# LeoIV/polyaxon

Hardware: AMD Instinct MI355X
Metric: HPO trials/hour (whole node) + wall-clock-to-target, ResNet-50 Hyperband sweep (higher is better)
Workload: dtype bf16

## Files before the change

polyaxon_amd/csrc/conv_gemm.hip:

```cpp
#include <hip/hip_runtime.h>

#include <stdint.h>

namespace {

typedef __bf16 bf16x8 __attribute__((ext_vector_type(8)));
typedef short s16x4 __attribute__((ext_vector_type(4)));
typedef float f32x4 __attribute__((ext_vector_type(4)));
typedef uint32_t u32x4 __attribute__((ext_vector_type(4)));
typedef __attribute__((address_space(3))) void lds_void;
typedef __attribute__((address_space(1))) const void gbl_void;

constexpr int BK = 64;

struct ConvGeom {
    int H, W;
    int Hr, Wr;
    int C, S, ntaps;
    int Hc, Wc, OS, oph, opw;
    signed char offh[9], offw[9], btap[9];
    int tap_a[9], tap_b[9];
    uint32_t mWr, mHr;
    int nh, nw, hv[3], wv[3];
    uint32_t pat[9];
    int tap_inner;
};

__device__ __forceinline__ int pick9(const int (&v)[9], int t) {
    int r = v[0];
#pragma unroll
    for (int i = 1; i < 9; ++i) r = t == i ? v[i] : r;
    return r;
}

inline uint32_t div_magic(int d) { return d <= 1 ? 0u : (uint32_t)((1ull << 32) / (unsigned)d + 1); }
// ... 606 lines not shown
    }
    if (stats_on) {
        float* pa = stats + (size_t)srow * N + n0;
        float* pb = stats + (size_t)(nsr + srow) * N + n0;
        reduce_store(s1, s2, pa, pb);
        zero_rows(pa, pb, N);
    }
}

template <int ROWB>
__device__ __forceinline__ int tr_swz(int row) {
    if constexpr (ROWB >= 256) return 2 * ((row & 3) | (((row >> 3) & 1) << 2));
    else return 2 * (((row >> 1) & 1) | (((row >> 3) & 1) << 1));
}

template <int ROWB>
__device__ __forceinline__ s16x4 tr_read(const char* img, int row, int col ) {
    const int lc = col >> 3, half = (col >> 2) & 1;
    const int pc = lc ^ tr_swz<ROWB>(row);
    return __builtin_amdgcn_ds_read_tr16_b64_v4i16(
        (__attribute__((address_space(3))) s16x4*)(img + row * ROWB + pc * 16 + half * 8));
}

__device__ __forceinline__ uint32_t lds_addr(const void* p) {
    return (uint32_t)(uintptr_t)(const __attribute__((address_space(3))) char*)p;
}

__device__ __forceinline__ s16x4 ds_tr(uint32_t addr) {
    s16x4 r;
    asm volatile("ds_read_b64_tr_b16 %0, %1" : "=v"(r) : "v"(addr) : "memory");
    return r;
}

template <int ROWB, int GATHER = 0, int BKR = BK>
__device__ __forceinline__ void stage_rows(char* img, __amdgpu_buffer_rsrc_t rsrc, int ld, int r0, int rend, int c0,
                                           int wave, int lane, const ConvGeom* geo = nullptr, int dh = 0, int dw = 0) {
    constexpr int INSTR = BKR * ROWB / 1024;
    static_assert(INSTR % 4 == 0, "a stage splits evenly over the 4 waves");
#pragma unroll
    for (int i = 0; i < INSTR / 4; ++i) {
        const int off = (i * 4 + wave) * 1024 + lane * 16;
        const int row = off / ROWB, pc = (off % ROWB) >> 4;
        const int lc = pc ^ tr_swz<ROWB>(row);
        const int gr = r0 + row;
        uint32_t boff;
        if constexpr (GATHER == 2) {
            int n, r, c;
            row_coords(gr, *geo, n, r, c);
            const int t = (c0 >> 3) + lc, ih = 2 * r - 3 + (t >> 2), sc = c - 2 + (t & 3);
            const bool ok = gr < rend && t < 28 && (unsigned)ih < (unsigned)geo->H && (unsigned)sc < (unsigned)geo->W;
            boff = ok ? (uint32_t)(((n * geo->H + ih) * geo->W + sc) * 16) : OOB;
        } else if constexpr (GATHER == 1) {
            int n, r, c;
            row_coords(gr, *geo, n, r, c);
            const int ih = r * geo->S + dh, iw = c * geo->S + dw;
            const bool ok = gr < rend && (unsigned)ih < (unsigned)geo->H && (unsigned)iw < (unsigned)geo->W;
            boff = ok ? (uint32_t)(((((n * geo->H + ih) * geo->W + iw) * ld) + c0 + lc * 8) * 2) : OOB;
        } else {
            boff = gr < rend ? (uint32_t)((gr * ld + c0 + lc * 8) * 2) : OOB;
        }
        blds16(rsrc, boff, img + (i * 4 + wave) * 1024);
    }
}


template <int BN1, int BN2, int WG1, int WG2, int CONV, int NST = 2, int BKT = BK>
// ... 357 lines not shown
            const float v = red[tw * 4096 + row * 64 + (lane ^ (((row >> 2) & 3) << 4))];
            float* dst = W + (size_t)(n10 + (tw / NB) * 64 + row) * ldc + n20 + (tw % NB) * 64 + lane;
            __hip_atomic_fetch_add(dst, v, __ATOMIC_RELAXED, __HIP_MEMORY_SCOPE_AGENT);
        }
        return;
    }
    float* slab = W + (size_t)slice * N1 * N2;
#pragma unroll
    for (int a = 0; a < 4; ++a)
#pragma unroll
        for (int b = 0; b < 4; ++b) {
            const int c2 = n20 + w2 * 64 + b * 16 + gi;
            const int r1 = n10 + w1 * 64 + a * 16 + 4 * g4;
#pragma unroll
            for (int r = 0; r < 4; ++r) slab[(size_t)(r1 + r) * N2 + c2] = acc[a][b][r];
        }
}

__global__ void weight_prep_kernel(const float* __restrict__ w, __bf16* __restrict__ wb, __bf16* __restrict__ wt,
                                   int cout, int cin) {
    __shared__ float tile[32][33];
    const int c0 = blockIdx.x * 32, o0 = blockIdx.y * 32;
    const int tx = threadIdx.x & 31, ty = threadIdx.x >> 5;
    for (int j = ty; j < 32; j += 8) {
        const int o = o0 + j, c = c0 + tx;
        float v = (o < cout && c < cin) ? w[(size_t)o * cin + c] : 0.f;
        tile[j][tx] = v;
        if (o < cout && c < cin) wb[(size_t)o * cin + c] = (__bf16)v;
    }
    __syncthreads();
    for (int j = ty; j < 32; j += 8) {
        const int c = c0 + j, o = o0 + tx;
        if (o < cout && c < cin) wt[(size_t)c * cout + o] = (__bf16)tile[tx][j];
    }
}

template <typename KernelT>
int set_lds(KernelT k, int bytes) {
    return hipFuncSetAttribute((const void*)k, hipFuncAttributeMaxDynamicSharedMemorySize, bytes) == hipSuccess ? 0
                                                                                                                 : -2;
}

template <int BM, int BN, int WGM, int WGN, int CONV = 0, int NBUF = 2>
int launch_nt(const void* A, const void* B, void* C, int M, int N, int K, int lda, int ldb, int ldc, float* stats,
              hipStream_t s, ConvGeom geo = {}, const void* D = nullptr, int ldd = 0, BnBwd bnr = {},
              const uint8_t* dmask = nullptr) {
    constexpr int NTH = NTHREADS;
    constexpr int TILE = BM * (BN * 2 + 16), RED = NTH * 17 * 4;
    constexpr int EPI = TILE > RED ? TILE : RED;
    constexpr int KLOOP = NBUF * (BM + BN) * BK * 2;
    constexpr int LDS = KLOOP > EPI ? KLOOP : EPI;
    static_assert(NBUF >= 1 && NBUF <= 2, "one or two K stages");
    static_assert(NBUF == 1 || EPI <= KLOOP, "epilogue staging must fit the k-loop LDS");
    static_assert(LDS <= 160 * 1024, "LDS");
    constexpr int PER_CU = (160 * 1024) / LDS;
    constexpr int CAP = CONV != 0 && BN == 64 ? 3 : 4;
    constexpr int MIN_F = NBUF == 1 ? (PER_CU < CAP ? PER_CU : CAP) : 2, MIN_B = MIN_F;
    auto kf = gemm_nt_kernel<BM, BN, WGM, WGN, CONV, MIN_F, NBUF, false, NTH>;
    auto kb = gemm_nt_kernel<BM, BN, WGM, WGN, CONV, MIN_B, NBUF, true, NTH>;
    static int attr = set_lds(kf, LDS) | set_lds(kb, LDS);
    if (attr) return attr;
    const bool bwd = D != nullptr || bnr.part != nullptr;
    if (bwd && stats != nullptr) return -1;
    auto k = bwd ? kb : kf;
    const int nwg = ((M + BM - 1) / BM) * (N / BN);
    hipLaunchKernelGGL(k, dim3(nwg), dim3(NTH), LDS, s, (const __bf16*)A, (const __bf16*)B, (__bf16*)C, M, N,
                       K, lda, ldb, ldc, stats, geo, (const __bf16*)D, ldd, bnr, dmask, BnDx{}, BnApply{});
    return hipGetLastError() == hipSuccess ? 0 : -3;
}

template <int BM, int BN, int WGM, int WGN, bool BNDX, int BNAP>
int launch_nt_prod(const void* A, const BnDx& bd, const BnApply& ba, const void* B, void* C, int M, int N, int K,
                   int ldb, int ldc, float* stats, hipStream_t s, const void* D = nullptr, int ldd = 0, BnBwd bnr = {},
                   const uint8_t* dmask = nullptr) {
    constexpr int TILE = BM * (BN * 2 + 16), RED = NTHREADS * 17 * 4;
    constexpr int LDS = 2 * (BM + BN) * BK * 2;
    static_assert(TILE <= LDS && RED <= LDS && LDS <= 80 * 1024, "epilogue staging fits; 2 blocks per CU");
    static_assert(BNDX != (BNAP != 0), "exactly one producer mode");
    auto k = gemm_nt_kernel<BM, BN, WGM, WGN, 0, 2, 2, BNDX, NTHREADS, BNDX, BNAP>;
    static int attr = set_lds(k, LDS);
    if (attr) return attr;
    const int nwg = ((M + BM - 1) / BM) * (N / BN);
    hipLaunchKernelGGL(k, dim3(nwg), dim3(NTHREADS), LDS, s, (const __bf16*)A, (const __bf16*)B, (__bf16*)C, M, N, K, K,
                       ldb, ldc, stats, ConvGeom{}, (const __bf16*)D, ldd, bnr, dmask, bd, ba);
    return hipGetLastError() == hipSuccess ? 0 : -3;
}


inline bool nt_single(bool conv, int K, int nwg) { return nwg >= 768 || (!conv && K == BK); }

inline int nt_plan(bool conv, int M, int N, int K) {
    const int bm = N % 128 == 0 ? 128 : 256, bn = N % 128 == 0 ? 128 : 64;
    return bm + 1000 * (nt_single(conv, K, ((M + bm - 1) / bm) * (N / bn)) ? 1 : 2);
}

struct TnPlan { int kchunk, slices, groups, per_group, blocks, bn1, bn2; };

inline void tn_tile(int N1, int N2, int& bn1, int& bn2) {
    bn1 = N1 % 128 == 0 ? 128 : 64;
    bn2 = N2 % 128 == 0 ? 128 : 64;
}

inline void plan_reducer(TnPlan& p, long plane) {
    const long total4 = plane / 4;
    int blocks = (int)((total4 + 255) / 256);
    if (blocks > 2048) blocks = 2048;
    int groups = 1024 / blocks;
    if (groups > p.slices / 8) groups = p.slices / 8;
    if (groups < 1) groups = 1;
    const int per_group = (p.slices + groups - 1) / groups;
    p.groups = (p.slices + per_group - 1) / per_group;
    p.per_group = per_group;
    p.blocks = blocks;
}

inline long plan_slabs(const TnPlan& p) { return p.slices + (p.groups > 1 ? p.groups : 0); }

constexpr int g_tn_bpc_big = 3, g_tn_bpc_mid = 1;
constexpr long g_tn_slab_bytes = 16l << 20;

// ... 161 lines not shown
    switch (nt_plan(false, M, N, K)) {
        case 1128:
            return launch_nt<128, 128, 2, 2, false, 1>(A, B, C, M, N, K, lda, ldb, ldc, stats, s, {}, D, ldd, b, dmask);
        case 2128:
            return launch_nt<128, 128, 2, 2>(A, B, C, M, N, K, lda, ldb, ldc, stats, s, {}, D, ldd, b, dmask);
        case 1256:
            return launch_nt<256, 64, 4, 1, false, 1>(A, B, C, M, N, K, lda, ldb, ldc, stats, s, {}, D, ldd, b, dmask);
        default:
            return launch_nt<256, 64, 4, 1>(A, B, C, M, N, K, lda, ldb, ldc, stats, s, {}, D, ldd, b, dmask);
    }
}

int plx_gemm_nt_plan(int M, int N, int K, int conv) {
    if (M <= 0 || N <= 0 || N % 64 || K <= 0 || K % BK) return -1;
    return nt_plan(conv != 0, M, N, K);
}

int plx_gemm_nt_bndx(const void* g, const void* x, const uint8_t* mask, const float* coef, void* dy, const void* Wt,
                     void* C, int M, int N, int K, int ldb, int ldc, const void* D, int ldd, const uint8_t* dmask,
                     const BnBwd* bnr, void* stream) {
    if (M <= 0 || N % 64 || K % BK || ldb % 8 || ldc % 8 || (D != nullptr && ldd % 8)) return -1;
    if (g == nullptr || x == nullptr || coef == nullptr || dy == nullptr || dy == g || dy == x) return -1;
    if ((long)M * K >= (1l << 30)) return -1;
    if (dmask != nullptr && (D == nullptr || ldd != N)) return -1;
    if (bnr != nullptr && (ldc != N || bnr->part == nullptr)) return -1;
    const BnBwd b = bnr != nullptr ? *bnr : BnBwd{};
    const BnDx bd{(const __bf16*)x, mask, coef, (__bf16*)dy};
    hipStream_t s = (hipStream_t)stream;
    if (N % 128 == 0)
        return launch_nt_prod<128, 128, 2, 2, true, 0>(g, bd, {}, Wt, C, M, N, K, ldb, ldc, nullptr, s, D, ldd, b, dmask);
    return launch_nt_prod<256, 64, 4, 1, true, 0>(g, bd, {}, Wt, C, M, N, K, ldb, ldc, nullptr, s, D, ldd, b, dmask);
}

int plx_gemm_nt_bnapply(const void* x, const void* res, const float* sb, const float* rsb, void* out, uint8_t* mask,
                        const void* W, void* C, int M, int N, int K, int ldb, int ldc, float* stats, void* stream) {
    if (M <= 0 || N % 64 || K % BK || ldb % 8 || ldc % 8) return -1;
    if (x == nullptr || res == nullptr || sb == nullptr || out == nullptr || mask == nullptr || out == x || out == res)
        return -1;
    if ((long)M * K >= (1l << 30)) return -1;
    const BnApply ba{(const __bf16*)res, sb, rsb, (__bf16*)out, mask};
    hipStream_t s = (hipStream_t)stream;
    if (N % 128 == 0)
        return rsb != nullptr ? launch_nt_prod<128, 128, 2, 2, false, 2>(x, {}, ba, W, C, M, N, K, ldb, ldc, stats, s)
                              : launch_nt_prod<128, 128, 2, 2, false, 1>(x, {}, ba, W, C, M, N, K, ldb, ldc, stats, s);
    return rsb != nullptr ? launch_nt_prod<256, 64, 4, 1, false, 2>(x, {}, ba, W, C, M, N, K, ldb, ldc, stats, s)
                          : launch_nt_prod<256, 64, 4, 1, false, 1>(x, {}, ba, W, C, M, N, K, ldb, ldc, stats, s);
}

int plx_tn_plan_slices(int M, int N1, int N2, int num_cus, int v2) {
    if (M <= 0 || N1 % 64 || N2 % 64) return -1;
    return v2 ? tn2_plan(M, N1, N2, num_cus, v2_cfg(N1, N2)).slices : tn_plan(M, N1, N2, num_cus).slices;
}

void plx_set_tn2_c64(int on) { g_tn2_c64 = on ? 1 : 0; }

void plx_set_tn_atomic(int on) { g_tn_atomic = on ? 1 : 0; }

void plx_set_tn2_stem(int mode) { g_tn2_stem = mode < 0 ? 0 : (mode > 2 ? 2 : mode); }

void plx_set_tn_v2(int on, int lds_kb) {
    g_tn_v2 = on < 0 ? 0 : (on > 2 ? 2 : on);
    if (lds_kb > 0) g_tn2_lds_kb = lds_kb <= 64 ? 64 : 128;
}

long plx_gemm_tn_workspace(int M, int N1, int N2, int num_cus) {
    if (M <= 0 || N1 % 64 || N2 % 64) return -1;
    const long a = plan_slabs(tn_plan(M, N1, N2, num_cus));
    const long b = plan_slabs(tn2_plan(M, N1, N2, num_cus, v2_cfg(N1, N2)));
    return (a > b ? a : b) * N1 * N2;
}

}

namespace {
template <int CONV>
int run_tn(const void* A, const void* B, float* C, float* ws, int M, int N1, int N2, int lda, int ldb, int ldc,
           int num_cus, int accumulate, hipStream_t s, ConvGeom geo, int bpc = 0) {
    const V2Cfg cfg = v2_cfg(N1, N2);
    const bool six = cfg.na == 1 && cfg.nb == 3;
    const bool v2 = CONV == 2 ? g_tn2_stem > 0
                              : (g_tn_v2 == 1 || (g_tn_v2 == 2 && CONV != 0)) && (!six || g_tn2_c64);
    const TnPlan plan = v2 ? tn2_plan(M, N1, N2, num_cus, cfg, CONV == 2 && g_tn2_stem == 1 ? kStemV2Bpc : 0)
                           : tn_plan(M, N1, N2, num_cus, bpc);
    int rc;
    if (v2 && g_tn_atomic) {
        if (!accumulate && hipMemset2DAsync(C, (size_t)ldc * 4, 0, (size_t)N2 * 4, N1, s) != hipSuccess) return -3;
        return dispatch_tn2<CONV>(cfg, A, B, C, M, N1, N2, lda, ldb, plan, s, geo, true, ldc);
    }
    if (v2)
// ... 330 lines not shown
```

polyaxon_amd/ops/_native.py:

```python
from __future__ import annotations

import ctypes
import hashlib
import os
import shutil
import subprocess
import threading
from pathlib import Path
from typing import Dict, Iterable, List, Optional

PKG_DIR = Path(__file__).resolve().parent.parent
CSRC = PKG_DIR / "csrc"
OUT = PKG_DIR / "_native"
ARCH = os.environ.get("PLX_OFFLOAD_ARCH", "gfx950")
ROCM = Path(os.environ.get("ROCM_PATH", "/opt/rocm"))

LIBRARIES: Dict[str, dict] = {
    "plx_train": {"sources": ["train_kernels.hip"], "kind": "hip", "link": []},
    "plx_polytune": {"sources": ["polytune_kernels.hip"], "kind": "hip", "link": []},
    "plx_bn": {"sources": ["bn_kernels.hip"], "kind": "hip", "link": []},
    "plx_procmon": {"sources": ["procmon.cpp"], "kind": "cpp", "link": ["-lpthread"]},
    "plx_gp": {"sources": ["gp_kernels.hip", "gp_chol.hip"], "kind": "hip", "link": []},
    "plx_rms": {"sources": ["rmsnorm.hip"], "kind": "hip", "link": []},
    "plx_conv": {"sources": ["conv_gemm.hip"], "kind": "hip", "link": []},
# ... 190 lines not shown
        "plx_bn_backward": [_P, _P],
        "plx_bn_dx_blocks": [_L, _I],
        "plx_stem_bn_pool_forward": [_P, _P, _P, _I, _I, _I, _I, _P, _P, _F, _F, _P, _P, _P, _P, _P, _P, _P, _I, _P,
                                     _P],
        "plx_stem_bn_pool_bwd_workspace": [_I, _I, _I, _I],
        "plx_stem_bn_pool_backward": [_P, _P, _P, _P, _I, _I, _I, _I, _P, _P, _P, _P, _P, _P, _P, _P, _I, _P, _P],
    },
    "plx_procmon": {
        "plx_pm_create": [],
        "plx_pm_destroy": [_P],
        "plx_pm_spawn": [_P, _P, _P, ctypes.c_char_p, ctypes.c_char_p, ctypes.POINTER(_I)],
        "plx_pm_wait": [_P, _I, ctypes.POINTER(_I), ctypes.POINTER(_I)],
        "plx_pm_wake": [_P],
        "plx_pm_signal": [_P, _I, _I, _I],
        "plx_pm_count": [_P],
    },
    "plx_gp": {
        "plx_gp_kmat": [_P, _P, _I, _I, _I, _P, _I, _I, _F, _F, _F, _I, _F, _P, _P, _D, _I, _P],
        "plx_gp_chol": [_P, _I, _I, _P, _P],
        "plx_gp_kmat_batch_f64": [_P, _I, _I, _P, _I, _P, _I, _L, _I, _D, _D, _D, _P, _P, _D, _I, _P],
        "plx_gp_matern_table": [_D, _D, _D, _I, _P, _P, _P],
        "plx_gp_chol_aug_f64": [_P, _I, _I, _I, _L, _I, _P, _P, _P],
        "plx_gp_chol_scratch_doubles": [],
        "plx_gp_lml_f64": [_P, _I, _I, _L, _I, _P, _P, _P],
        "plx_gp_acq_rows": [_P, _I, _I, _P, _F, _I, _F, _F, _F, _P, _P, _P, _P],
        "plx_gp_predict_acq": [_P, _I, _P, _I, _I, _P, _I, _P, _I, _F, _F, _F, _F, _I, _F, _F, _F, _P, _P, _P, _P,
                               _P, _P, _P, _D, _I, _P],
        "plx_gp_ascent": [_P, _P, _I, _P, _P, _P, _I, _I, _P, _P, _I, _F, _F, _F, _F, _I, _F, _F, _F, _I, _P, _P, _D, _I,
                          _P],
    },
    "plx_conv": {
        "plx_gemm_nt": [_P, _P, _P, _I, _I, _I, _I, _I, _I, _P, _P, _I, _P, _P, _P],
        "plx_gemm_nt_bndx": [_P, _P, _P, _P, _P, _P, _P, _I, _I, _I, _I, _I, _P, _I, _P, _P, _P],
        "plx_gemm_nt_bnapply": [_P, _P, _P, _P, _P, _P, _P, _P, _I, _I, _I, _I, _I, _P, _P],
        "plx_gemm_nt_rows_per_block": [_I],
        "plx_gemm_nt_plan": [_I, _I, _I, _I],
        "plx_gemm_tn_workspace": [_I, _I, _I, _I],
        "plx_set_tn_v2": [_I, _I],
        "plx_set_tn2_stem": [_I],
        "plx_set_tn2_c64": [_I],
        "plx_set_tn_atomic": [_I],
        "plx_tn_plan_slices": [_I, _I, _I, _I, _I],
        "plx_gemm_tn": [_P, _P, _P, _P, _I, _I, _I, _I, _I, _I, _I, _I, _P],
        "plx_weight_prep": [_P, _P, _P, _I, _I, _P],
        "plx_weight_prepk": [_P, _L, _L, _L, _L, _P, _P, _I, _I, _I, _P],
        "plx_weight_prep_all": [_P, _P, _P, _P, _I, _I, _P],
        "plx_stem_pack_input": [_P, _P, _I, _I, _I, _P],
        "plx_stem_pack_weight": [_P, _L, _L, _L, _L, _P, _I, _P],
        "plx_stem_conv_fwd": [_P, _P, _P, _I, _I, _I, _P, _P],
        "plx_stem_conv_wgrad_workspace": [_I, _I, _I, _I],
        "plx_stem_conv_wgrad": [_P, _P, _P, _L, _L, _L, _L, _P, _I, _I, _I, _I, _I, _P],
        "plx_conv_fwd": [_P, _P, _P, _I, _I, _I, _I, _I, _I, _I, _P, _P],
        "plx_conv_dgrad": [_P, _P, _P, _I, _I, _I, _I, _I, _I, _I, _P, _P, _P],
        "plx_conv_dgrad_blocks": [_I, _I, _I, _I, _I, _I, _I],
        "plx_conv_wgrad_workspace": [_I, _I, _I, _I, _I, _I, _I, _I],
        "plx_conv_wgrad": [_P, _P, _P, _P, _I, _I, _I, _I, _I, _I, _I, _I, _I, _P],
    },
    "plx_lm": {
        "plx_qkv_rope_fwd": [_P, _P, _P, _P, _P, _P, _L, _I, _I, _I, _I, _I, _P],
        "plx_qkv_rope_bwd": [_P, _P, _P, _P, _P, _P, _L, _I, _I, _I, _I, _I, _P],
        "plx_swiglu_fwd": [_P, _P, _L, _I, _P],
        "plx_swiglu_bwd": [_P, _P, _P, _L, _I, _P],
        "plx_xent_fwd": [_P, _P, _P, _P, _I, _I, _I, _P],
        "plx_xent_bwd": [_P, _P, _P, _P, _P, _I, _I, _I, _P],
        "plx_xent_cls_fwd": [_P, _P, _P, _P, _I, _I, _P],
        "plx_xent_cls_bwd": [_P, _P, _P, _P, _P, _I, _I, _F, _P],
        "plx_xent_hp_fwd": [_P, _P, _P, _P, _P, _P, _I, _I, _I, _I, _P],
        "plx_xent_hp_bwd": [_P, _P, _P, _P, _P, _P, _I, _I, _I, _I, _P],
        "plx_xent_cls_hp_fwd": [_P, _P, _P, _P, _P, _P, _I, _I, _I, _P],
        "plx_xent_cls_hp_bwd": [_P, _P, _P, _P, _P, _P, _I, _I, _I, _F, _P],
        "plx_colsum_splits": [_L, _I],
        "plx_colsum": [_P, _L, _I, _P, _P, _P, _I, _P],
        "plx_gelu_bwd_colsum": [_P, _P, _P, _L, _I, _P, _P, _P, _I, _P],
    },
# ... 107 lines not shown
```

polyaxon_amd/ops/conv1x1.py:

```python
from __future__ import annotations

import ctypes
import os
from typing import Dict

import torch
import torch.nn as nn
import torch.nn.functional as F

from polyaxon_amd.ops import _native, side_stream, wcache
from polyaxon_amd.ops.flat import direct_grad

_CUS: Dict[int, int] = {}

_BN_DX_FUSED = os.environ.get("PLX_BN_DX_FUSED", "1") != "0"


def set_bn_dx_fused(on: bool) -> bool:
    global _BN_DX_FUSED
    prev, _BN_DX_FUSED = _BN_DX_FUSED, bool(on)
    return prev


_BN_APPLY_FUSED = os.environ.get("PLX_BN_APPLY_FUSED", "1") != "0"


def set_bn_apply_fused(on: bool) -> bool:
    global _BN_APPLY_FUSED
    prev, _BN_APPLY_FUSED = _BN_APPLY_FUSED, bool(on)
    return prev


def bn_apply_fused() -> bool:
    return _BN_APPLY_FUSED


def _num_cus(dev: torch.device) -> int:
    idx = dev.index if dev.index is not None else torch.cuda.current_device()
    if idx not in _CUS:
        _CUS[idx] = torch.cuda.get_device_properties(idx).multi_processor_count
    return _CUS[idx]


def _stream() -> int:
    return _native.current_stream()


def nt_stats_rows(n: int) -> int:
    return _native.size("plx_conv", "plx_gemm_nt_rows_per_block", n)


def _check_stats(stats, m: int, n: int) -> None:
    if stats is not None:
        nblk = -(-m // nt_stats_rows(n))
        assert stats.dtype == torch.float32 and stats.is_contiguous() and stats.numel() >= 2 * nblk * n


def _check_add(add, add_mask, m: int, n: int) -> None:
    if add is not None:
        assert add.shape == (m, n) and add.stride(1) == 1 and add.dtype == torch.bfloat16 and add.data_ptr() % 16 == 0
    if add_mask is not None:
        assert add is not None and add.stride(0) == n and add_mask.dtype == torch.uint8 and add_mask.numel() == m * n // 8


def gemm_nt(a: torch.Tensor, b: torch.Tensor, out: torch.Tensor = None, stats: torch.Tensor = None,
            add: torch.Tensor = None, bnr: "_native.GemmBnBwdArgs" = None,
            add_mask: torch.Tensor = None) -> torch.Tensor:
# ... 9 lines not shown
                                             b.stride(0), out.stride(0),
                                             stats.data_ptr() if stats is not None else None,
                                             add.data_ptr() if add is not None else None,
                                             add.stride(0) if add is not None else 0,
                                             add_mask.data_ptr() if add_mask is not None else None,
                                             ctypes.addressof(bnr) if bnr is not None else None, _stream())
    _native.check(rc, "plx_gemm_nt")
    return out


def gemm_nt_bndx(g: torch.Tensor, x: torch.Tensor, mask: torch.Tensor, coef: torch.Tensor, dy: torch.Tensor,
                 b: torch.Tensor, out: torch.Tensor = None, add: torch.Tensor = None,
                 bnr: "_native.GemmBnBwdArgs" = None, add_mask: torch.Tensor = None) -> torch.Tensor:
    m, k = g.shape
    n = b.shape[0]
    if out is None:
        out = torch.empty(m, n, dtype=torch.bfloat16, device=g.device)
    for t in (g, x, dy):
        assert t.shape == (m, k) and t.dtype == torch.bfloat16 and t.stride() == (k, 1) and t.data_ptr() % 16 == 0
    assert b.stride(1) == 1 and out.stride(1) == 1 and b.shape[1] == k and b.dtype == torch.bfloat16
    assert b.data_ptr() % 16 == 0 and out.data_ptr() % 16 == 0
    assert coef.dtype == torch.float32 and coef.is_contiguous() and coef.numel() == 3 * k
    if mask is not None:
        assert mask.dtype == torch.uint8 and mask.numel() == m * k // 8
    _check_add(add, add_mask, m, n)
    rc = _native.lib("plx_conv").plx_gemm_nt_bndx(g.data_ptr(), x.data_ptr(),
                                                  mask.data_ptr() if mask is not None else None, coef.data_ptr(),
                                                  dy.data_ptr(), b.data_ptr(), out.data_ptr(), m, n, k, b.stride(0),
                                                  out.stride(0), add.data_ptr() if add is not None else None,
                                                  add.stride(0) if add is not None else 0,
                                                  add_mask.data_ptr() if add_mask is not None else None,
                                                  ctypes.addressof(bnr) if bnr is not None else None, _stream())
    _native.check(rc, "plx_gemm_nt_bndx")
    return out


def gemm_nt_bnapply(x: torch.Tensor, res: torch.Tensor, sb: torch.Tensor, rsb, out_a: torch.Tensor, mask: torch.Tensor,
                    b: torch.Tensor, out: torch.Tensor = None, stats: torch.Tensor = None) -> torch.Tensor:
    m, k = x.shape
    n = b.shape[0]
    if out is None:
        out = torch.empty(m, n, dtype=torch.bfloat16, device=x.device)
    for t in (x, res, out_a):
        assert t.shape == (m, k) and t.dtype == torch.bfloat16 and t.stride() == (k, 1) and t.data_ptr() % 16 == 0
    assert b.stride(1) == 1 and out.stride(1) == 1 and b.shape[1] == k and b.dtype == torch.bfloat16
    assert b.data_ptr() % 16 == 0 and out.data_ptr() % 16 == 0
    assert mask.dtype == torch.uint8 and mask.is_contiguous() and mask.numel() >= m * k // 8
    for c in (sb, rsb):
        assert c is None or (c.dtype == torch.float32 and c.is_contiguous() and c.numel() == 2 * k
                             and c.data_ptr() % 16 == 0)
    assert sb is not None
    _check_stats(stats, m, n)
    rc = _native.lib("plx_conv").plx_gemm_nt_bnapply(x.data_ptr(), res.data_ptr(), sb.data_ptr(),
                                                     rsb.data_ptr() if rsb is not None else None, out_a.data_ptr(),
                                                     mask.data_ptr(), b.data_ptr(), out.data_ptr(), m, n, k,
                                                     b.stride(0), out.stride(0),
                                                     stats.data_ptr() if stats is not None else None, _stream())
    _native.check(rc, "plx_gemm_nt_bnapply")
    return out


def gemm_tn(a: torch.Tensor, b: torch.Tensor, out: torch.Tensor = None, accumulate: bool = False) -> torch.Tensor:
    m, n1 = a.shape
    n2 = b.shape[1]
    if out is None:
        out = torch.empty(n1, n2, dtype=torch.float32, device=a.device)
# ... 201 lines not shown
        x = x.to(torch.bfloat16).contiguous(memory_format=torch.channels_last)
        ctx.box = box
        ctx.dxsink = dxsink
        ctx.sink = sink if (sink is not None and sink.armed) else None
        if ctx.sink is not None:
            ctx.sink.expect = True
        ctx.link = link if (sink is None or sink.armed) else None
        ctx.wgrad = direct_grad(weight)
        n, cin, h, w = x.shape
        cout = weight.shape[0]
        wb, wt = wcache.lookup(weight) or weight_prep(weight)
        y = torch.empty((n, cout, h, w), dtype=torch.bfloat16, device=x.device, memory_format=torch.channels_last)
        if pend is not None:
            gemm_nt_bnapply(_rows(pend.x), _rows(pend.res), pend.sb, pend.rsb, _rows(x), pend.mask, wb, _rows(y), stats)
            pend.release()
        else:
            gemm_nt(_rows(x), wb, _rows(y), stats)
        ctx.save_for_backward(x, wt)
        ctx.wshape = weight.shape
        ctx.wdtype = weight.dtype
        return y

    @staticmethod
    def backward(ctx, dy):
        x, wt = ctx.saved_tensors
        n, cin, h, w = x.shape
        fused = ctx.dxsink.take() if ctx.dxsink is not None else None
        if fused is not None and (dy.data_ptr() != fused[4].data_ptr() or dy.shape != fused[4].shape
                                  or dy.dtype != torch.bfloat16 or not ctx.needs_input_grad[0]):
            raise RuntimeError("DxSink: the BatchNorm's deferred input gradient was replaced before the convolution's "
                               "backward could fill it")
        dy = dy.to(torch.bfloat16).contiguous(memory_format=torch.channels_last)
        dx = dw = None
        extra, extra_mask = ctx.box.take() if ctx.box is not None else (None, None)
        if ctx.needs_input_grad[0]:
            dx = torch.empty_like(x, memory_format=torch.channels_last)
            if extra is not None and (extra.dtype != torch.bfloat16
                                      or not extra.is_contiguous(memory_format=torch.channels_last)):
                if extra_mask is not None:
                    extra, extra_mask = unpack_relu_mask(extra, extra_mask), None
                extra = extra.to(torch.bfloat16).contiguous(memory_format=torch.channels_last)
            bnr = None
            rows = nt_stats_rows(cin)
            if ctx.link is not None and ctx.sink is None and (ctx.box is None or extra is not None):
                bnr = ctx.link.request(-(-(n * h * w) // rows))
            elif ctx.link is not None and ctx.sink is not None and ctx.sink.s2k1 and extra is None:
                bnr = ctx.link.request_split(-(-(n * h * w) // rows), -(-(n * ((h + 1) // 2) * ((w + 1) // 2)) // rows))
            if fused is not None:
                g, bx, bmask, coef, _ = fused
                gemm_nt_bndx(_rows(g), _rows(bx), bmask, coef, _rows(dy), wt, _rows(dx),
                             add=_rows(extra) if extra is not None else None, bnr=bnr, add_mask=extra_mask)
            else:
                gemm_nt(_rows(dy), wt, _rows(dx), add=_rows(extra) if extra is not None else None, bnr=bnr,
                        add_mask=extra_mask)
            if ctx.sink is not None:
                ctx.sink.put(dx)
                dx = None
        if ctx.needs_input_grad[1]:
            cout = ctx.wshape[0]
            if ctx.wgrad is not None:
                slot = ctx.wgrad.as_strided((cout, cin), (cin, 1))
                side_stream.run(lambda: gemm_tn(_rows(dy), _rows(x), out=slot, accumulate=True), (dy, x), x.device)
            else:
                dw = gemm_tn(_rows(dy), _rows(x)).view(ctx.wshape).to(ctx.wdtype)
        return dx, dw, None, None, None, None, None, None


def _bf16_context(x: torch.Tensor) -> bool:
    if x.dtype == torch.bfloat16:
        return True
    return torch.is_autocast_enabled("cuda") and torch.get_autocast_dtype("cuda") == torch.bfloat16


def supported(x: torch.Tensor, conv: nn.Conv2d) -> bool:
    return (x.is_cuda and x.dim() == 4 and _bf16_context(x) and conv.kernel_size == (1, 1) and conv.stride == (1, 1)
            and conv.padding == (0, 0) and conv.groups == 1 and conv.bias is None
            and conv.in_channels % 64 == 0 and conv.out_channels % 64 == 0 and x.numel() > 0)


def conv1x1(x: torch.Tensor, weight: torch.Tensor, with_stats: bool = False,
            grad_box: "GradMailbox" = None, grad_sink: "GradMailbox" = None, bn_link: bool = False) -> torch.Tensor:
    stats = None
    if with_stats:
        n, _, h, w = x.shape
        m, cout = n * h * w, weight.shape[0]
        nblk = -(-m // nt_stats_rows(cout))
        stats = torch.empty(2 * nblk * cout, dtype=torch.float32, device=x.device)
    if grad_box is not None:
        grad_box.armed = True
    dxsink = dx_sink_for(x, weight)
    pend = getattr(x, "_plx_pending", None)
# ... 31 lines not shown
```

Before: 13000.

## Fuse weight-gradient accumulation into BN-dx producer dgrad kernel for 64-channel 1x1 convs

Adds a persistent kernel for 1x1 convs with 64 input channels. It rebuilds the BatchNorm input gradient tile once in LDS and uses it for both the data-gradient GEMM and the weight-gradient product against the saved input. The weight gradient is reduced in registers across row tiles and flushed with atomic adds into the fp32 weight-grad buffer. This removes the separate gemm_tn pass that re-read dy and x, but that pass used to run on a side stream and now runs serially inside the dgrad kernel, so the overlap is lost and the dgrad kernel does more work. It is on by default through an environment flag, but only when the atomic weight-gradient mode is enabled.

```diff
diff --git a/polyaxon_amd/csrc/conv_gemm.hip b/polyaxon_amd/csrc/conv_gemm.hip
--- a/polyaxon_amd/csrc/conv_gemm.hip
+++ b/polyaxon_amd/csrc/conv_gemm.hip
@@ -1,6 +1,8 @@
 #include <hip/hip_runtime.h>
 
 #include <stdint.h>
+
+#include <type_traits>
 
 namespace {
 
@@ -673,6 +675,14 @@
     return r;
 }
 
+template <int OFF>
+__device__ __forceinline__ s16x4 ds_tr_o(uint32_t addr) {
+    static_assert(OFF >= 0 && OFF < 65536, "16-bit offset field");
+    s16x4 r;
+    asm volatile("ds_read_b64_tr_b16 %0, %1 offset:%2" : "=v"(r) : "v"(addr), "n"(OFF) : "memory");
+    return r;
+}
+
 template <int ROWB, int GATHER = 0, int BKR = BK>
 __device__ __forceinline__ void stage_rows(char* img, __amdgpu_buffer_rsrc_t rsrc, int ld, int r0, int rend, int c0,
                                            int wave, int lane, const ConvGeom* geo = nullptr, int dh = 0, int dw = 0) {
@@ -1096,6 +1106,349 @@
     for (int j = ty; j < 32; j += 8) {
         const int c = c0 + j, o = o0 + tx;
         if (o < cout && c < cin) wt[(size_t)c * cout + o] = (__bf16)tile[tx][j];
+    }
+}
+
+template <int NK>
+__global__ void __launch_bounds__(512, 1)
+bndx_wgrad_kernel(const __bf16* __restrict__ G, const __bf16* __restrict__ B, __bf16* __restrict__ C, int M, int ldb,
+                  int ldc, const __bf16* __restrict__ D, int ldd, BnBwd bnr, const uint8_t* __restrict__ dmask, BnDx bd,
+                  const __bf16* __restrict__ Xin, float* __restrict__ dW, int lddw) {
+    constexpr int BM = 256, BN = 64, NW = 8, K = NK * BK;
+    constexpr int A_BYTES = BM * BK * 2, B_BYTES = BN * BK * 2, STAGE = A_BYTES + B_BYTES;
+    constexpr int XOFF = 2 * STAGE;
+    constexpr int AI = BM / (8 * NW);
+    extern __shared__ __attribute__((aligned(16))) char smem[];
+
+    const int ntm = (M + BM - 1) / BM;
+    if ((int)blockIdx.x >= ntm) return;
+    const int tid = threadIdx.x, lane = tid & 63;
+    const int wave = __builtin_amdgcn_readfirstlane(tid >> 6);
+    const int fr = lane & 15, fq = lane >> 4;
+
+    const int srow = wave * 8 + (lane >> 3);
+    const int lc8 = ((lane & 7) ^ tr_swz<128>(srow)) * 8;
+    const uint32_t b_off = (uint32_t)((srow * ldb + ((lane & 7) ^ nt_swz(srow)) * 8) * 2);
+    const __amdgpu_buffer_rsrc_t rg = buf_rsrc(G), rb = buf_rsrc(B), rx = buf_rsrc(bd.x), rc = buf_rsrc(bd.coef),
+                                 rxi = buf_rsrc(Xin);
+    uint32_t e_off[AI];
+    u32x4 gq[AI], xq[AI];
+    uint32_t mq[AI];
+    u32x4 cf[6];
+    auto set_tile = [&](int m0) {
+#pragma unroll
+        for (int i = 0; i < AI; ++i) {
+            const int gm = m0 + i * 64 + srow;
+            e_off[i] = gm < M ? (uint32_t)((gm * K + lc8) * 2) : OOB;
+        }
+    };
+    auto stage_x = [&](int m0) {
+#pragma unroll
+        for (int i = 0; i < AI; ++i) {
+            const int gm = m0 + i * 64 + srow;
+            blds16(rxi, gm < M ? (uint32_t)((gm * BN + lc8) * 2) : OOB, smem + XOFF + (i * NW + wave) * 1024);
+        }
+    };
+    auto stage_b = [&](int buf, int k0) { blds16(rb, b_off + (uint32_t)(k0 * 2), smem + buf * STAGE + A_BYTES + wave * 1024); };
+    auto load_a = [&](int k0) {
+#pragma unroll
+        for (int i = 0; i < AI; ++i) {
+            gq[i] = __builtin_amdgcn_raw_buffer_load_b128(rg, (int)e_off[i], k0 * 2, 0);
+            xq[i] = __builtin_amdgcn_raw_buffer_load_b128(rx, (int)e_off[i], k0 * 2, 0);
+        }
+        if (bd.mask != nullptr) {
+            const __amdgpu_buffer_rsrc_t rm = buf_rsrc(bd.mask);
+#pragma unroll
+            for (int i = 0; i < AI; ++i)
+                mq[i] = __builtin_amdgcn_raw_buffer_load_b8(rm, (int)(e_off[i] == OOB ? OOB : e_off[i] >> 4), k0 >> 3, 0);
+        } else {
+#pragma unroll
+            for (int i = 0; i < AI; ++i) mq[i] = 0xffu;
+        }
+#pragma unroll
+        for (int r = 0; r < 3; ++r) {
+            cf[2 * r] = __builtin_amdgcn_raw_buffer_load_b128(rc, lc8 * 4, (r * K + k0) * 4, 0);
+            cf[2 * r + 1] = __builtin_amdgcn_raw_buffer_load_b128(rc, lc8 * 4 + 16, (r * K + k0) * 4, 0);
+        }
+    };
+    auto xform_a = [&](int buf) {
+        char* base = smem + buf * STAGE;
+        const float* ca = (const float*)&cf[0];
+        const float* cb = (const float*)&cf[2];
+        const float* cd = (const float*)&cf[4];
+#pragma unroll
+        for (int i = 0; i < AI; ++i) {
+            const uint32_t* pg = (const uint32_t*)&gq[i];
+            const uint32_t* px = (const uint32_t*)&xq[i];
+            u32x4 o;
+            uint32_t* po = (uint32_t*)&o;
+            const uint32_t mb = mq[i];
+#pragma unroll
+            for (int j = 0; j < 4; ++j) {
+                const float g0 = (mb >> (2 * j)) & 1u ? __uint_as_float(pg[j] << 16) : 0.f;
+                const float g1 = (mb >> (2 * j + 1)) & 1u ? __uint_as_float(pg[j] & 0xffff0000u) : 0.f;
+                const float x0 = __uint_as_float(px[j] << 16), x1 = __uint_as_float(px[j] & 0xffff0000u);
+                const float o0 = fmaf(ca[2 * j], g0, fmaf(cb[2 * j], x0, cd[2 * j]));
+                const float o1 = fmaf(ca[2 * j + 1], g1, fmaf(cb[2 * j + 1], x1, cd[2 * j + 1]));
+                po[j] = pack_bf16x2(o0, o1);
+            }
+            if (e_off[i] == OOB) o = u32x4{0u, 0u, 0u, 0u};
+            *(u32x4*)(base + (i * NW + wave) * 1024 + lane * 16) = o;
+        }
+    };
+
+    f32x4 accw[NK][2];
+#pragma unroll
+    for (int a = 0; a < NK; ++a) accw[a][0] = accw[a][1] = f32x4{0.f, 0.f, 0.f, 0.f};
+    const int kt4 = wave >> 1, nt2 = (wave & 1) * 2;
+    const int trow = 8 * fq + (fr >> 2), tcol = 4 * (fr & 3);
+    auto tr_off = [&](int col) {
+        return (uint32_t)(trow * 128 + (((col >> 3) ^ tr_swz<128>(trow)) << 4) + ((col >> 2) & 1) * 8);
+    };
+    const uint32_t wa_off = tr_off(kt4 * 16 + tcol), wx_off0 = tr_off(nt2 * 16 + tcol), wx_off1 = tr_off(nt2 * 16 + 16 + tcol);
+
+    constexpr int CROW = BN * 2 + 16, CHUNKS = BN / 8, RSTEP = 256 / CHUNKS, ITERS = BM / RSTEP;
+    char* const ep = smem + STAGE;
+    const bool bnr_on = bnr.part != nullptr, d_on = D != nullptr;
+
+    int tm = blockIdx.x;
+    set_tile(tm * BM);
+    stage_x(tm * BM);
+    load_a(0);
+    stage_b(0, 0);
+    for (; tm < ntm; tm += gridDim.x) {
+        const int m0 = tm * BM;
+        f32x4 acc[4][2];
+#pragma unroll
+        for (int a = 0; a < 4; ++a) acc[a][0] = acc[a][1] = f32x4{0.f, 0.f, 0.f, 0.f};
+        xform_a(0);
+        asm volatile("s_waitcnt vmcnt(0)" ::: "memory");
+        __syncthreads();
+#pragma unroll
+        for (int kt = 0; kt < NK; ++kt) {
+            const int cur = kt & 1;
+            if (kt + 1 < NK) {
+                load_a((kt + 1) * BK);
+                stage_b(cur ^ 1, (kt + 1) * BK);
+            }
+            const char* As = smem + cur * STAGE;
+            const char* Bs = As + A_BYTES;
+#pragma unroll
+            for (int kk = 0; kk < 2; ++kk) {
+                bf16x8 fa[4], fb[2];
+#pragma unroll
+                for (int rn = 0; rn < 4; ++rn) {
+                    const int row = rn * 16 + fr;
+                    fa[rn] = *(const bf16x8*)(Bs + row * 128 + (((kk * 4 + fq) ^ nt_swz(row)) << 4));
+                }
+#pragma unroll
+                for (int rm = 0; rm < 2; ++rm) {
+                    const int row = wave * 32 + rm * 16 + fr;
+                    fb[rm] = *(const bf16x8*)(As + row * 128 + (((kk * 4 + fq) ^ tr_swz<128>(row)) << 4));
+                }
+#pragma unroll
+                for (int rn = 0; rn < 4; ++rn)
+#pragma unroll
+                    for (int rm = 0; rm < 2; ++rm)
+                        acc[rn][rm] = __builtin_amdgcn_mfma_f32_16x16x32_bf16(fa[rn], fb[rm], acc[rn][rm], 0, 0, 0);
+            }
+            const uint32_t sa_ = lds_addr(As) + wa_off;
+            const uint32_t sx_[2] = {lds_addr(smem + XOFF) + wx_off0, lds_addr(smem + XOFF) + wx_off1};
+            auto dw_steps = [&](auto msc) {
+                constexpr int O = decltype(msc)::value * 32 * 128;
+                s16x4 alo[2], ahi[2], xlo[2][2], xhi[2][2];
+                alo[0] = ds_tr_o<O>(sa_);
+                ahi[0] = ds_tr_o<O + 512>(sa_);
+                alo[1] = ds_tr_o<O + 4096>(sa_);
+                ahi[1] = ds_tr_o<O + 4608>(sa_);
+#pragma unroll
+                for (int j = 0; j < 2; ++j) {
+                    xlo[0][j] = ds_tr_o<O>(sx_[j]);
+                    xhi[0][j] = ds_tr_o<O + 512>(sx_[j]);
+                    xlo[1][j] = ds_tr_o<O + 4096>(sx_[j]);
+                    xhi[1][j] = ds_tr_o<O + 4608>(sx_[j]);
+                }
+                asm volatile("s_waitcnt lgkmcnt(0)"
+                             : "+v"(alo[0]), "+v"(ahi[0]), "+v"(alo[1]), "+v"(ahi[1]), "+v"(xlo[0][0]), "+v"(xhi[0][0]),
+                               "+v"(xlo[0][1]), "+v"(xhi[0][1]), "+v"(xlo[1][0]), "+v"(xhi[1][0]), "+v"(xlo[1][1]),
+                               "+v"(xhi[1][1]));
+#pragma unroll
+                for (int u = 0; u < 2; ++u) {
+                    const bf16x8 fw = __builtin_bit_cast(bf16x8, __builtin_shufflevector(alo[u], ahi[u], 0, 1, 2, 3, 4, 5, 6, 7));
+#pragma unroll
+                    for (int j = 0; j < 2; ++j) {
+                        const bf16x8 fx =
+                            __builtin_bit_cast(bf16x8, __builtin_shufflevector(xlo[u][j], xhi[u][j], 0, 1, 2, 3, 4, 5, 6, 7));
+                        accw[kt][j] = __builtin_amdgcn_mfma_f32_16x16x32_bf16(fw, fx, accw[kt][j], 0, 0, 0);
+                    }
+                }
+            };
+            dw_steps(std::integral_constant<int, 0>{});
+            dw_steps(std::integral_constant<int, 2>{});
+            dw_steps(std::integral_constant<int, 4>{});
+            dw_steps(std::integral_constant<int, 6>{});
+            __builtin_amdgcn_sched_barrier(0);
+            if (kt + 1 < NK) xform_a(cur ^ 1);
+            asm volatile("s_waitcnt vmcnt(0)" ::: "memory");
+            __syncthreads();
+        }
+        const int tnext = tm + gridDim.x;
+        if (tnext < ntm) {
+            set_tile(tnext * BM);
+            stage_x(tnext * BM);
+            load_a(0);
+            stage_b(0, 0);
+        }
+        const int rows = min(BM, M - m0);
+        int te = tid;
+        asm volatile("" : "+v"(te));
+        const int cc = te % CHUNKS, ch0 = cc * 8;
+        const bool ep_thread = te < 256;
+#pragma unroll
+        for (int rm = 0; rm < 2; ++rm) {
+            const int ml = wave * 32 + rm * 16 + fr;
+#pragma unroll
+            for (int rn = 0; rn < 4; ++rn) {
+                const f32x4 v = acc[rn][rm];
+                uint2 packed;
+                packed.x = pack_bf16x2(v[0], v[1]);
+                packed.y = pack_bf16x2(v[2], v[3]);
+                *(uint2*)(ep + ml * CROW + (rn * 16 + fq * 4) * 2) = packed;
+            }
+        }
+        __syncthreads();
+        {
+            constexpr int AIT = BM / 64;
+            const int ra0 = te / CHUNKS;
+            int orow[AIT];
+            uint4 dpre[AIT];
+            uint32_t dmpre[AIT];
+#pragma unroll
+            for (int i = 0; i < AIT; ++i) orow[i] = min(m0 + ra0 + i * 64, M - 1);
+            if (d_on) {
+#pragma unroll
+                for (int i = 0; i < AIT; ++i) dpre[i] = *(const uint4*)(D + (size_t)orow[i] * ldd + ch0);
+                if (dmask != nullptr) {
+#pragma unroll
+                    for (int i = 0; i < AIT; ++i) dmpre[i] = dmask[((size_t)orow[i] * ldd + ch0) >> 3];
+                }
+            }
+#pragma unroll
+            for (int i = 0; i < AIT; ++i) {
+                const int r = ra0 + i * 64;
+                if (r >= rows) break;
+                uint4 v = *(const uint4*)(ep + r * CROW + cc * 16);
+                if (d_on) {
+                    uint32_t* pv = (uint32_t*)&v;
+                    const uint32_t* pd = (const uint32_t*)&dpre[i];
+                    const uint32_t db = dmask != nullptr ? dmpre[i] : 0xffu;
+#pragma unroll
+                    for (int j = 0; j < 4; ++j) {
+                        const float d0 = (db >> (2 * j)) & 1u ? __uint_as_float(pd[j] << 16) : 0.f;
+                        const float d1 = (db >> (2 * j + 1)) & 1u ? __uint_as_float(pd[j] & 0xffff0000u) : 0.f;
+                        const float lo = __uint_as_float(pv[j] << 16) + d0;
+                        const float hi = __uint_as_float(pv[j] & 0xffff0000u) + d1;
+                        pv[j] = pack_bf16x2(lo, hi);
+                    }
+                    if (bnr_on) *(uint4*)(ep + r * CROW + cc * 16) = v;
+                }
+                *(uint4*)(C + (size_t)orow[i] * ldc + ch0) = v;
+            }
+        }
+        float sa[8], sb[8];
+        if (bnr_on) {
+            __syncthreads();
+            if (ep_thread) {
+                const int r0 = te / CHUNKS;
+                float mu[8], is[8];
+#pragma unroll
+                for (int k = 0; k < 8; ++k) {
+                    sa[k] = sb[k] = 0.f;
+                    mu[k] = bnr.mean[ch0 + k];
+                    is[k] = bnr.invstd[ch0 + k];
+                }
+#pragma unroll
+                for (int h = 0; h < 2; ++h) {
+                    constexpr int HI = ITERS / 2;
+                    asm volatile("" ::: "memory");
+                    uint4 xpre[HI];
+                    uint32_t mpre[HI];
+#pragma unroll
+                    for (int i = 0; i < HI; ++i) {
+                        const size_t e = (size_t)min(m0 + r0 + (h * HI + i) * RSTEP, M - 1) * ldc + ch0;
+                        xpre[i] = *(const uint4*)(bnr.x + e);
+                        mpre[i] = bnr.mask != nullptr ? bnr.mask[e >> 3] : 0xffu;
+                    }
+                    if (bnr.skip_w > 0) {
+#pragma unroll
+                        for (int i = 0; i < HI; ++i) {
+                            const int gm = m0 + r0 + (h * HI + i) * RSTEP, q = gm / bnr.skip_w;
+                            if (((gm - q * bnr.skip_w) | (q % bnr.skip_h)) % 2 == 0) mpre[i] = 0u;
+                        }
+                    }
+#pragma unroll
+                    for (int i = 0; i < HI; ++i) {
+                        const int r = r0 + (h * HI + i) * RSTEP;
+                        if (r >= rows) break;
+                        const uint4 v = *(const uint4*)(ep + r * CROW + cc * 16);
+                        const uint32_t mb = mpre[i];
+                        const uint32_t* pv = (const uint32_t*)&v;
+                        const uint32_t* px = (const uint32_t*)&xpre[i];
+#pragma unroll
+                        for (int j = 0; j < 4; ++j) {
+                            const float g0 = (mb >> (2 * j)) & 1u ? __uint_as_float(pv[j] << 16) : 0.f;
+                            const float g1 = (mb >> (2 * j + 1)) & 1u ? __uint_as_float(pv[j] & 0xffff0000u) : 0.f;
+                            const float x0 = __uint_as_float(px[j] << 16), x1 = __uint_as_float(px[j] & 0xffff0000u);
+                            sa[2 * j] += g0;
+                            sa[2 * j + 1] += g1;
+                            sb[2 * j] = fmaf(g0, (x0 - mu[2 * j]) * is[2 * j], sb[2 * j]);
+                            sb[2 * j + 1] = fmaf(g1, (x1 - mu[2 * j + 1]) * is[2 * j + 1], sb[2 * j + 1]);
+                        }
+                    }
+                }
+            }
+        }
+        if (bnr_on) {
+            float* red = (float*)ep;
+            __syncthreads();
+            if (ep_thread) {
+#pragma unroll
+                for (int k = 0; k < 8; ++k) {
+                    red[te * 17 + k] = sa[k];
+                    red[te * 17 + 8 + k] = sb[k];
+                }
+            }
+            __syncthreads();
+            if (te < CHUNKS * 16) {
+                const int c = te % CHUNKS, v = te / CHUNKS;
+                float sum = 0.f;
+#pragma unroll 4
+                for (int j = 0; j < RSTEP; ++j) sum += red[(j * CHUNKS + c) * 17 + v];
+                float* pa = bnr.part + (size_t)(bnr.blk_off + tm) * ldc;
+                float* pb = bnr.part + (size_t)(bnr.part_ld + bnr.blk_off + tm) * ldc;
+                if (v < 8) pa[c * 8 + v] = sum;
+                else pb[c * 8 + v - 8] = sum;
+            }
+        }
+    }
+    asm volatile("s_waitcnt vmcnt(0)" ::: "memory");
+    __syncthreads();
+    float* red = (float*)smem;
+    static_assert(K * 256 <= 2 * STAGE, "the flush image fits the stage buffers");
+#pragma unroll
+    for (int kt = 0; kt < NK; ++kt)
+#pragma unroll
+        for (int j = 0; j < 2; ++j)
+#pragma unroll
+            for (int r = 0; r < 4; ++r) {
+                const int row = kt * 64 + kt4 * 16 + 4 * fq + r, col = (nt2 + j) * 16 + fr;
+                red[row * 64 + (col ^ (((row >> 2) & 3) << 4))] = accw[kt][j][r];
+            }
+    __syncthreads();
+#pragma unroll 4
+    for (int row = wave; row < K; row += NW) {
+        const float v = red[row * 64 + (lane ^ (((row >> 2) & 3) << 4))];
+        __hip_atomic_fetch_add(dW + (size_t)row * lddw + lane, v, __ATOMIC_RELAXED, __HIP_MEMORY_SCOPE_AGENT);
     }
 }
 
@@ -1150,6 +1503,29 @@
     return hipGetLastError() == hipSuccess ? 0 : -3;
 }
 
+template <int NK>
+int launch_bndx_wgrad(const void* g, const BnDx& bd, const void* Wt, void* C, int M, int ldb, int ldc, const void* D,
+                      int ldd, const BnBwd& bnr, const uint8_t* dmask, const void* x_in, float* dW, int lddw, int blocks,
+                      hipStream_t s) {
+    constexpr int LDS = 2 * (256 + 64) * BK * 2 + 256 * 64 * 2;
+    static_assert(LDS <= 160 * 1024, "LDS");
+    auto k = bndx_wgrad_kernel<NK>;
+    static int attr = set_lds(k, LDS);
+    if (attr) return attr;
+    int grid = blocks;
+    if (grid <= 0) {
+        int dev = 0, cus = 0;
+        if (hipGetDevice(&dev) != hipSuccess ||
+            hipDeviceGetAttribute(&cus, hipDeviceAttributeMultiprocessorCount, dev) != hipSuccess || cus <= 0)
+            return -3;
+        const int ntm = (M + 255) / 256;
+        grid = cus < ntm ? cus : ntm;
+    }
+    hipLaunchKernelGGL(k, dim3(grid), dim3(512), LDS, s, (const __bf16*)g, (const __bf16*)Wt, (__bf16*)C, M, ldb, ldc,
+                       (const __bf16*)D, ldd, bnr, dmask, bd, (const __bf16*)x_in, dW, lddw);
+    return hipGetLastError() == hipSuccess ? 0 : -3;
+}
+
 
 inline bool nt_single(bool conv, int K, int nwg) { return nwg >= 768 || (!conv && K == BK); }
 
@@ -1377,6 +1753,28 @@
     return launch_nt_prod<256, 64, 4, 1, true, 0>(g, bd, {}, Wt, C, M, N, K, ldb, ldc, nullptr, s, D, ldd, b, dmask);
 }
 
+int plx_gemm_nt_bndx_wgrad(const void* g, const void* x, const uint8_t* mask, const float* coef, void* dy,
+                           const void* Wt, void* C, int M, int N, int K, int ldb, int ldc, const void* D, int ldd,
+                           const uint8_t* dmask, const BnBwd* bnr, const void* x_in, float* dW, int lddw, int blocks,
+                           void* stream) {
+    (void)dy;
+    if (M <= 0 || N != 64 || K % BK || K < BK || K > 4 * BK || ldb % 8 || ldc % 8 || (D != nullptr && ldd % 8)) return -1;
+    if (g == nullptr || x == nullptr || coef == nullptr || x_in == nullptr || dW == nullptr || lddw < N || blocks < 0)
+        return -1;
+    if ((long)M * K >= (1l << 30)) return -1;
+    if (dmask != nullptr && (D == nullptr || ldd != N)) return -1;
+    if (bnr != nullptr && (ldc != N || bnr->part == nullptr)) return -1;
+    const BnBwd b = bnr != nullptr ? *bnr : BnBwd{};
+    const BnDx bd{(const __bf16*)x, mask, coef, nullptr};
+    hipStream_t s = (hipStream_t)stream;
+    switch (K / BK) {
+        case 1: return launch_bndx_wgrad<1>(g, bd, Wt, C, M, ldb, ldc, D, ldd, b, dmask, x_in, dW, lddw, blocks, s);
+        case 2: return launch_bndx_wgrad<2>(g, bd, Wt, C, M, ldb, ldc, D, ldd, b, dmask, x_in, dW, lddw, blocks, s);
+        case 3: return launch_bndx_wgrad<3>(g, bd, Wt, C, M, ldb, ldc, D, ldd, b, dmask, x_in, dW, lddw, blocks, s);
+        default: return launch_bndx_wgrad<4>(g, bd, Wt, C, M, ldb, ldc, D, ldd, b, dmask, x_in, dW, lddw, blocks, s);
+    }
+}
+
 int plx_gemm_nt_bnapply(const void* x, const void* res, const float* sb, const float* rsb, void* out, uint8_t* mask,
                         const void* W, void* C, int M, int N, int K, int ldb, int ldc, float* stats, void* stream) {
     if (M <= 0 || N % 64 || K % BK || ldb % 8 || ldc % 8) return -1;
@@ -1400,6 +1798,8 @@
 void plx_set_tn2_c64(int on) { g_tn2_c64 = on ? 1 : 0; }
 
 void plx_set_tn_atomic(int on) { g_tn_atomic = on ? 1 : 0; }
+
+int plx_get_tn_atomic() { return g_tn_atomic; }
 
 void plx_set_tn2_stem(int mode) { g_tn2_stem = mode < 0 ? 0 : (mode > 2 ? 2 : mode); }
 
diff --git a/polyaxon_amd/ops/_native.py b/polyaxon_amd/ops/_native.py
--- a/polyaxon_amd/ops/_native.py
+++ b/polyaxon_amd/ops/_native.py
@@ -246,6 +246,7 @@
     "plx_conv": {
         "plx_gemm_nt": [_P, _P, _P, _I, _I, _I, _I, _I, _I, _P, _P, _I, _P, _P, _P],
         "plx_gemm_nt_bndx": [_P, _P, _P, _P, _P, _P, _P, _I, _I, _I, _I, _I, _P, _I, _P, _P, _P],
+        "plx_gemm_nt_bndx_wgrad": [_P, _P, _P, _P, _P, _P, _P, _I, _I, _I, _I, _I, _P, _I, _P, _P, _P, _P, _I, _I, _P],
         "plx_gemm_nt_bnapply": [_P, _P, _P, _P, _P, _P, _P, _P, _I, _I, _I, _I, _I, _P, _P],
         "plx_gemm_nt_rows_per_block": [_I],
         "plx_gemm_nt_plan": [_I, _I, _I, _I],
@@ -254,6 +255,7 @@
         "plx_set_tn2_stem": [_I],
         "plx_set_tn2_c64": [_I],
         "plx_set_tn_atomic": [_I],
+        "plx_get_tn_atomic": [],
         "plx_tn_plan_slices": [_I, _I, _I, _I, _I],
         "plx_gemm_tn": [_P, _P, _P, _P, _I, _I, _I, _I, _I, _I, _I, _I, _P],
         "plx_weight_prep": [_P, _P, _P, _I, _I, _P],
diff --git a/polyaxon_amd/ops/conv1x1.py b/polyaxon_amd/ops/conv1x1.py
--- a/polyaxon_amd/ops/conv1x1.py
+++ b/polyaxon_amd/ops/conv1x1.py
@@ -33,6 +33,20 @@
 
 def bn_apply_fused() -> bool:
     return _BN_APPLY_FUSED
+
+
+_DGRAD_WGRAD_FUSED = os.environ.get("PLX_DGRAD_WGRAD_FUSED", "1") != "0"
+
+
+def set_dgrad_wgrad_fused(on: bool) -> bool:
+    global _DGRAD_WGRAD_FUSED
+    prev, _DGRAD_WGRAD_FUSED = _DGRAD_WGRAD_FUSED, bool(on)
+    return prev
+
+
+def dgrad_wgrad_fused_ok(cin: int, cout: int) -> bool:
+    return (_DGRAD_WGRAD_FUSED and cin == 64 and cout <= 256 and cout % 64 == 0
+            and bool(_native.lib("plx_conv").plx_get_tn_atomic()))
 
 
 def _num_cus(dev: torch.device) -> int:
@@ -108,6 +122,37 @@
                                                   add_mask.data_ptr() if add_mask is not None else None,
                                                   ctypes.addressof(bnr) if bnr is not None else None, _stream())
     _native.check(rc, "plx_gemm_nt_bndx")
+    return out
+
+
+def gemm_nt_bndx_wgrad(g: torch.Tensor, x: torch.Tensor, mask: torch.Tensor, coef: torch.Tensor, dy: torch.Tensor,
+                       b: torch.Tensor, x_in: torch.Tensor, dw: torch.Tensor, out: torch.Tensor = None,
+                       add: torch.Tensor = None, bnr: "_native.GemmBnBwdArgs" = None, add_mask: torch.Tensor = None,
+                       blocks: int = 0) -> torch.Tensor:
+    m, k = g.shape
+    n = b.shape[0]
+    if out is None:
+        out = torch.empty(m, n, dtype=torch.bfloat16, device=g.device)
+    for t in (g, x, dy):
+        assert t.shape == (m, k) and t.dtype == torch.bfloat16 and t.stride() == (k, 1) and t.data_ptr() % 16 == 0
+    assert b.stride(1) == 1 and out.stride(1) == 1 and b.shape[1] == k and b.dtype == torch.bfloat16
+    assert b.data_ptr() % 16 == 0 and out.data_ptr() % 16 == 0
+    assert coef.dtype == torch.float32 and coef.is_contiguous() and coef.numel() == 3 * k
+    if mask is not None:
+        assert mask.dtype == torch.uint8 and mask.numel() == m * k // 8
+    assert x_in.shape == (m, n) and x_in.dtype == torch.bfloat16 and x_in.stride() == (n, 1) and x_in.data_ptr() % 16 == 0
+    assert dw.shape == (k, n) and dw.dtype == torch.float32 and dw.stride(1) == 1
+    _check_add(add, add_mask, m, n)
+    rc = _native.lib("plx_conv").plx_gemm_nt_bndx_wgrad(g.data_ptr(), x.data_ptr(),
+                                                        mask.data_ptr() if mask is not None else None,
+                                                        coef.data_ptr(), dy.data_ptr(), b.data_ptr(), out.data_ptr(),
+                                                        m, n, k, b.stride(0), out.stride(0),
+                                                        add.data_ptr() if add is not None else None,
+                                                        add.stride(0) if add is not None else 0,
+                                                        add_mask.data_ptr() if add_mask is not None else None,
+                                                        ctypes.addressof(bnr) if bnr is not None else None,
+                                                        x_in.data_ptr(), dw.data_ptr(), dw.stride(0), blocks, _stream())
+    _native.check(rc, "plx_gemm_nt_bndx_wgrad")
     return out
 
 
@@ -375,6 +420,7 @@
                                "backward could fill it")
         dy = dy.to(torch.bfloat16).contiguous(memory_format=torch.channels_last)
         dx = dw = None
+        wgrad_done = False
         extra, extra_mask = ctx.box.take() if ctx.box is not None else (None, None)
         if ctx.needs_input_grad[0]:
             dx = torch.empty_like(x, memory_format=torch.channels_last)
@@ -389,7 +435,15 @@
                 bnr = ctx.link.request(-(-(n * h * w) // rows))
             elif ctx.link is not None and ctx.sink is not None and ctx.sink.s2k1 and extra is None:
                 bnr = ctx.link.request_split(-(-(n * h * w) // rows), -(-(n * ((h + 1) // 2) * ((w + 1) // 2)) // rows))
-            if fused is not None:
+            cout = ctx.wshape[0]
+            if (fused is not None and ctx.needs_input_grad[1] and ctx.wgrad is not None
+                    and dgrad_wgrad_fused_ok(cin, cout)):
+                g, bx, bmask, coef, _ = fused
+                gemm_nt_bndx_wgrad(_rows(g), _rows(bx), bmask, coef, _rows(dy), wt, _rows(x),
+                                   ctx.wgrad.as_strided((cout, cin), (cin, 1)), _rows(dx),
+                                   add=_rows(extra) if extra is not None else None, bnr=bnr, add_mask=extra_mask)
+                wgrad_done = True
+            elif fused is not None:
                 g, bx, bmask, coef, _ = fused
                 gemm_nt_bndx(_rows(g), _rows(bx), bmask, coef, _rows(dy), wt, _rows(dx),
                              add=_rows(extra) if extra is not None else None, bnr=bnr, add_mask=extra_mask)
@@ -399,7 +453,7 @@
             if ctx.sink is not None:
                 ctx.sink.put(dx)
                 dx = None
-        if ctx.needs_input_grad[1]:
+        if ctx.needs_input_grad[1] and not wgrad_done:
             cout = ctx.wshape[0]
             if ctx.wgrad is not None:
                 slot = ctx.wgrad.as_strided((cout, cin), (cin, 1))
```

Result: faster. 13140 (median of 6 runs) (+1.1%).
